# neel-dey/anatomix

Measured on AMD Instinct MI355X. Metric: 128^3 volumes/sec feature-extraction (6M UNet), higher is better.
Workload: dtype f16; 1 GPU; anatomix 6M UNet (ngf=16,num_downs=4) forward on sw_batch=4 windows of 1x128^3 (the predictor call of sliding_window_inference, BASELINE configs[1] / the metric); fp32 NCDHW in/out, 16-bit (f16) channels-last activations, fp32 accumulate; holds the 1e-3 tolerance against the fp32 reference in rel-L2 ONLY (max-norm 0.86e-3 .. 1.4e-3 by weight seed; the mode that holds both norms is value_strict); batch_per_gpu=4, window=128, parallelism=replicas x1 (no data-path collective)

## Files before the change

### anatomix_amd/csrc/amx_conv3d_zmarch.hip

```cpp
#include <stdio.h>
#include <stdlib.h>
#include <string.h>

#include "amx_device.h"

namespace amx {

typedef __attribute__((address_space(1))) const void* gptr_t;
typedef __attribute__((address_space(3))) void* lptr_t;

template <int NCK, int QT, int TY, int TX, int R>
struct ZmCfg {
  static constexpr int NC = 8, TZ = 2;
  static constexpr int NL = 2 * NCK;
  static constexpr int HY = TY + 2, HX = TX + 2, HVP = HY * HX;
  static constexpr int PPL = ((HVP * 16 + 255) / 256) * 256;
  static constexpr int PLSZ = NL * PPL;
  static constexpr int FLAGOFF = R * PLSZ;
  static constexpr int LDS_BYTES = R * PLSZ + 64;
  static constexpr int XT = TX / 16;
  static constexpr int WPQ = NC / QT;
  static constexpr int NDMA = (HVP + 63) / 64;
  static_assert(WPQ == (TY / 2) * XT, "each consumer wave owns a 2 x 2 x 16 voxel block per step");
  static_assert(R - 4 > TZ, "ring must hold more than one step of prefetch");
  static constexpr bool VMCNT_OK = R * NDMA <= 60;
  static_assert(NL <= 8 && LDS_BYTES <= 160 * 1024, "ring must fit the LDS");
};

template <int QT, int TY, int TX, int OUTMODE>
struct ZmStage {
  static constexpr int CB = 32 * QT;
  static constexpr int CS = 2 * TY * TX * 4 + 64;
  static constexpr int BYTES = OUTMODE == 0 ? 2 * TY * TX * CB : 16 * QT * CS;
  static constexpr int NB = OUTMODE == 0 ? 2 : 1;
  static constexpr int TOTAL = NB * BYTES;
};

struct StemIn {
  const char* src;
  long long sn, sz, sy;
  long long offs[16];
  int use_offs;
  const char* wpk;
  const float* bias;
  int act;
  float slope;
};

template <int TY, int TX>
struct ZmStemCfg {
  static constexpr int HY = TY + 2, HX = TX + 2, HVP = HY * HX;
  static constexpr int IY = HY + 2, IX = HX + 2, IVP = IY * IX;
  static constexpr int RS = (TX + 8) * 2;
  static constexpr int CPSZ = IY * RS;
  static constexpr int IPLSZ = ((2 * CPSZ + 8 + 63) / 64) * 64;
  static constexpr int DUMMY = IPLSZ - 8;
  static constexpr int RC = 16;
  static constexpr int SW = 40;
  static constexpr int STGSZ = ((IY * SW * 4 + 255) / 256) * 256;
  static constexpr int RSTG = 8;
  static constexpr int NLD = (IVP + 63) / 64;
  static constexpr int BYTES = RC * IPLSZ + RSTG * STGSZ;
  static constexpr int NSW = 7;
  static constexpr int LEAD = 3;
  static constexpr int NT = 2 * HY + (2 * HY + 15) / 16;
  static constexpr bool OK = TX == 32 && IY == 12 && RSTG * 2 <= 60 && NLD == 7;
};

template <typename T, int NCK, int QT, int TY, int TX, int R, int OUTMODE, int NS, bool POOL, bool SPLIT = false, bool STEM = false>
__global__ __launch_bounds__((8 + (STEM ? ZmStemCfg<8, 32>::NSW + 1 : 2 * (SPLIT ? 2 : NCK)) + NS) * 64) void conv3d_k3_zmarch_kernel(const ConvParams p, int zseg, int nseg, const StemIn si) {
  static_assert(!SPLIT || (NCK == 1 && QT == 1 && NS == 0), "strict z-march: 16 -> 16, direct stores");
  static_assert(!STEM || (NCK == 1 && !SPLIT && NS == 0 && OUTMODE == 0), "stem-fed z-march: 16 input channels, direct 16-bit stores");
  constexpr int NCKP = SPLIT ? 2 : NCK;
  typedef ZmCfg<NCKP, QT, TY, TX, R> C;
  typedef ZmStage<QT, TY, TX, OUTMODE> SG;
  typedef typename Ops<T>::vec8 vec8;
  constexpr int HX = C::HX, PPL = C::PPL, PLSZ = C::PLSZ, XT = C::XT, NDMA = C::NDMA, NL = C::NL, NC = C::NC, TZ = C::TZ;
  constexpr int STAGEOFF = C::FLAGOFF + 128;
  static_assert(NS == 0 || NS == 2, "one storer wave per output plane of a step");
  static_assert(NS == 0 || STAGEOFF + SG::TOTAL <= 160 * 1024, "ring + staging tile must fit the LDS");

  extern __shared__ __attribute__((aligned(16))) char smem[];

  const int tid = threadIdx.x, lane = tid & 63;
  const int wave = __builtin_amdgcn_readfirstlane(tid >> 6);

  int b = blockIdx.x;
  const int nb = gridDim.x;
  if ((nb & 7) == 0) b = (b & 7) * (nb >> 3) + (b >> 3);
  const int bx = b % p.nbx;
  b /= p.nbx;
  const int by = b % p.nby;
  b /= p.nby;
  const int sg = b % nseg;
  const int n = b / nseg;
  const int y0 = by * TY, x0 = bx * TX;
  const int zs = sg * zseg;
  const int ze = (zs + zseg < p.D) ? zs + zseg : p.D;
  const int nplanes = ze - zs + 2;
  const int nsteps = (ze - zs + TZ - 1) / TZ;

  int* ready = (int*)(smem + C::FLAGOFF);
  int* done = (int*)(smem + C::FLAGOFF + 32);
  int* staged = (int*)(smem + C::FLAGOFF + 64);
  int* stored = (int*)(smem + C::FLAGOFF + 96);
  if (tid < ((NS || STEM) ? 32 : 16))
    ((int*)(smem + C::FLAGOFF))[tid] = (STEM && (tid < 8 || tid >= 24)) ? ((tid & 7) == 7 ? 0x7fffffff : (tid & 7)) : 0;
  if constexpr (STEM) {
    typedef ZmStemCfg<TY, TX> SC;
    static_assert(SC::OK && STAGEOFF + SC::BYTES <= 160 * 1024, "stem-fed geometry; ring + input rings must fit the LDS");
    for (int i = tid; i < SC::RC * SC::IPLSZ / 4; i += (NC + SC::NSW + 1) * 64) ((int*)(smem + STAGEOFF))[i] = 0;
  }
  __syncthreads();

  if (NS && wave >= NC + NL) {
    const int w = wave - NC - NL;
    const unsigned a_staged = lds_addr(staged), a_stored = lds_addr(stored + w);
    if constexpr (OUTMODE == 0) {
      constexpr int NR = TY * QT;
      const char* sbase = smem + STAGEOFF + w * TY * TX * SG::CB + lane * 16;
      char* gbase = p.out + (long long)n * p.on + (long long)y0 * p.oy + (long long)x0 * p.ox + lane * 16;
      for (int s = 0; s < nsteps; ++s) {
        while (__builtin_amdgcn_readfirstlane(flag_min8_asm(a_staged)) < s + 1) __builtin_amdgcn_s_sleep(1);
        uint4 v[NR];
#pragma unroll
        for (int r = 0; r < NR; ++r) v[r] = *(const uint4*)(sbase + (s % SG::NB) * SG::BYTES + r * 1024);
        asm volatile("s_waitcnt lgkmcnt(0)" ::: "memory");
        flag_store_asm(a_stored, s + 1);
        const int zo = zs + s * TZ + w;
        if (zo >= ze || (p.dbg & 4)) continue;
        char* dst = gbase + (long long)zo * p.oz;
#pragma unroll
        for (int r = 0; r < NR; ++r) *(uint4*)(dst + (long long)(r / QT) * p.oy + (r % QT) * 1024) = v[r];
      }
    } else {
      constexpr int NCH = 16 * QT;
      const int y = lane >> 3, xq = lane & 7;
      const char* sbase = smem + STAGEOFF + (w * TY + y) * (TX * 4) + xq * 16;
      float* gbase = p.out32 + (long long)n * p.pn + (long long)(y0 + y) * p.py + x0 + xq * 4;
      for (int s = 0; s < nsteps; ++s) {
        while (__builtin_amdgcn_readfirstlane(flag_min8_asm(a_staged)) < s + 1) __builtin_amdgcn_s_sleep(1);
        float4 v[NCH];
#pragma unroll
        for (int c = 0; c < NCH; ++c) v[c] = *(const float4*)(sbase + c * SG::CS);
        asm volatile("s_waitcnt lgkmcnt(0)" ::: "memory");
        flag_store_asm(a_stored, s + 1);
        const int zo = zs + s * TZ + w;
        if (zo >= ze || (p.dbg & 4)) continue;
        float* dst = gbase + (long long)zo * p.pz;
        if (p.wmap) {
          const float4 wg = *(const float4*)(p.wmap + ((long long)zo * p.H + y0 + y) * p.W + x0 + xq * 4);
#pragma unroll
          for (int c = 0; c < NCH; ++c) {
            const float4 old = *(const float4*)(dst + (long long)c * p.pc);
            v[c] = make_float4(old.x + wg.x * v[c].x, old.y + wg.y * v[c].y, old.z + wg.z * v[c].z, old.w + wg.w * v[c].w);
          }
        }
#pragma unroll
        for (int c = 0; c < NCH; ++c) *(float4*)(dst + (long long)c * p.pc) = v[c];
      }
    }
    return;
  }

  if constexpr (STEM) {
    if (wave >= NC) {
      typedef ZmStemCfg<TY, TX> SC;
      constexpr int RS = SC::RS, CPSZ = SC::CPSZ, IPLSZ = SC::IPLSZ, RC = SC::RC, RSTG = SC::RSTG, NLD = SC::NLD, IX = SC::IX, SW = SC::SW;
      constexpr int INOFF = STAGEOFF, STGOFF = STAGEOFF + RC * IPLSZ;
      int* landed = staged;
      int* inconv = stored;
      const int zlo = zs >= 2 ? zs - 2 : 0;
      const int zhi = ze + 1 <= p.D - 1 ? ze + 1 : p.D - 1;
      const int nin = zhi - zlo + 1;
      const char* src_n = si.src + (si.use_offs ? si.offs[n & 15] : (long long)n * si.sn);
      if (wave == NC + SC::NSW) {
        const int pr = lane / 10, pc = lane - pr * 10;
        const bool pvalid = lane < 60;
        int goff[2];
#pragma unroll
        for (int j = 0; j < 2; ++j) {
          int yy = y0 - 2 + pr + 6 * j, xx = x0 - 4 + 4 * pc;
          yy = yy < 0 ? 0 : (yy > p.H - 1 ? p.H - 1 : yy);
          xx = xx < 0 ? 0 : (xx > p.W - 4 ? p.W - 4 : xx);
          goff[j] = pvalid ? yy * (int)si.sy + xx * 4 : 0;
        }
        auto issue_plane = [&](int k) {
          const char* plane = src_n + (long long)(zlo + k) * si.sz;
          char* dstp = smem + STGOFF + (k % RSTG) * SC::STGSZ;
          if (pvalid) {
            __builtin_amdgcn_global_load_lds((gptr_t)(plane + goff[0]), (lptr_t)dstp, 16, 0, 0);
            __builtin_amdgcn_global_load_lds((gptr_t)(plane + goff[1]), (lptr_t)(dstp + 960), 16, 0, 0);
          }
        };
        int next_issue = 0, next_pub = 0, seen_conv = 0;
        const unsigned a_landed = lds_addr(landed);
#ifdef AMX_EXPERIMENT
        unsigned long long* ltr = (p.dbg & 8) && lane == 0 && blockIdx.x == 0 ? (unsigned long long*)p.stats + 1001 * 128 : nullptr;
        int lcount = 0;
#define AMX_LSTAMP() do { if (ltr && lcount < 128) ltr[lcount] = __builtin_readcyclecounter(); ++lcount; } while (0)
        AMX_LSTAMP();
#else
#define AMX_LSTAMP() do {} while (0)
#endif
        while (next_pub < nin) {
          while (next_issue < nin) {
            const int need = next_issue - RSTG + 1;
            if (seen_conv < need) seen_conv = __builtin_amdgcn_readfirstlane(flag_min8_asm(lds_addr(inconv)));
            if (seen_conv < need) break;
            issue_plane(next_issue++);
          }
          if (next_issue == next_pub) {
            __builtin_amdgcn_s_sleep(2);
            continue;
          }
          AMX_LSTAMP();
          WaitVm<2, RSTG - 1>::run(next_issue - next_pub - 1);
          AMX_LSTAMP();
          flag_store_asm(a_landed, ++next_pub);
          AMX_LSTAMP();
        }
        return;
      }
      constexpr int NSW = SC::NSW;
      const int w = wave - NC;
      const int li = lane & 15, g = lane >> 4;
      const vec8 w0 = *(const vec8*)(si.wpk + 4096 + lane * 16);
      typedef __attribute__((ext_vector_type(2))) unsigned u32x2;
      typedef __attribute__((ext_vector_type(4))) unsigned u32x4;
      u32x2 w1 = *(const u32x2*)(si.wpk + 4096 + 1024 + lane * 16);
      if (g) w1 = u32x2{0u, 0u};
      const f32x4 sbias = si.bias ? *(const f32x4*)(si.bias + g * 4) : f32x4{0.f, 0.f, 0.f, 0.f};
      asm volatile("s_waitcnt vmcnt(0)" ::: "memory");
      const float lo_clip = si.act == ACT_RELU ? 0.f : -__builtin_inff();
      const int r0 = 2 * g, r1 = 2 * g + 1;
      const int kz0 = r0 / 3, kz1 = r1 / 3;
      auto xpart = [&](int hx) -> int {
        const int v0 = reflect_clamp(x0 + hx - 1, p.W) - (x0 - 2) - 1;
        return (v0 & 1) * CPSZ + (v0 & ~1) * 2;
      };
      auto ytop = [&](int hy) -> int { return reflect_clamp(y0 + hy - 1, p.H) - (y0 - 2) - 1; };
      const int xA = xpart(li), xB = xpart(16 + li);
      const int d0 = __builtin_amdgcn_readfirstlane((ytop(0) - 0) * RS), d9 = __builtin_amdgcn_readfirstlane((ytop(9) - 9) * RS);
      const int wlane = (g >> 1) * PPL + (g & 1) * 8 + li * 16;
      int croff[2], cwoff[2];
#pragma unroll
      for (int c = 0; c < 2; ++c) {
        const int crow = 8 * c + (li >> 1);
        const bool cvalid = crow < C::HY;
        const int crc = cvalid ? crow : 0;
        croff[c] = ytop(crc) * RS + xpart(32 + (li & 1));
        cwoff[c] = cvalid ? (g >> 1) * PPL + (g & 1) * 8 + (crow * HX + 32 + (li & 1)) * 16 : (g >> 1) * PPL + C::HVP * 16 + (g & 1) * 8;
      }
      constexpr int NB = 4;
      float vmax = 0.f;
      int seen_in = 0, seen_done = 0;
      int myk = w, seen_landed = 0, seen_ready = 0;
      bool ibad = false;
      auto convert_plane = [&](int k) {
        while (seen_landed < k + 1) {
          seen_landed = flag_load(landed);
          if (seen_landed < k + 1) __builtin_amdgcn_s_sleep(1);
        }
        const int need_done = zlo + k - RC + 3 - zs;
        while (seen_ready < need_done) {
          seen_ready = __builtin_amdgcn_readfirstlane(flag_min8_asm(lds_addr(ready)));
          if (seen_ready < need_done) __builtin_amdgcn_s_sleep(1);
        }
        asm volatile("" ::: "memory");
        const int so = (k % RSTG) * SC::STGSZ, dof = ((zlo + k) % RC) * IPLSZ;
        int lane_o = lane;
        asm volatile("" : "+v"(lane_o));
#pragma unroll
        for (int j = 0; j < NLD; ++j) {
          const int hv = j * 64 + lane_o;
          const bool valid = hv < SC::IVP;
          const int hvc = valid ? hv : SC::IVP - 1;
          const int iy = hvc / IX, ix = hvc - iy * IX;
          const int ry = reflect_clamp(y0 + iy - 2, p.H) - (y0 - 2), rx = reflect_clamp(x0 + ix - 2, p.W) - (x0 - 4);
          const float f = *(const float*)(smem + STGOFF + so + (ry * SW + rx) * 4);
          if (RangeCheck<T>::on) ibad |= RangeCheck<T>::bad(f);
          const unsigned short hb = to_bits<T>(f);
          const int la = valid ? iy * RS + ix * 2 : SC::DUMMY;
          const int lb = (valid && ix > 0) ? CPSZ + iy * RS + (ix - 1) * 2 : SC::DUMMY;
          *(unsigned short*)(smem + INOFF + dof + la) = hb;
          *(unsigned short*)(smem + INOFF + dof + lb) = hb;
        }
        asm volatile("" ::: "memory");
        flag_store(inconv + w, k + NSW);
      };
#ifdef AMX_EXPERIMENT
      unsigned long long* str = (p.dbg & 8) && lane == 0 && blockIdx.x == 0 && w == 0 ? (unsigned long long*)p.stats + 1000 * 128 : nullptr;
      int scount = 0;
#define AMX_SSTAMP() do { if (str && scount < 128) str[scount] = __builtin_readcyclecounter(); ++scount; } while (0)
      AMX_SSTAMP();
#else
#define AMX_SSTAMP() do {} while (0)
#endif
      for (int q = w; q < nplanes; q += NSW) {
        const int z1 = reflect_clamp(zs - 1 + q, p.D);
        int zi[3];
#pragma unroll
        for (int kz = 0; kz < 3; ++kz) zi[kz] = reflect_clamp(z1 - 1 + kz, p.D);
        int zmax = zi[0] > zi[1] ? zi[0] : zi[1];
        zmax = zmax > zi[2] ? zmax : zi[2];
        {
          int kmax = zs + q - zlo + SC::LEAD;
          kmax = kmax < nin - 1 ? kmax : nin - 1;
          for (; myk <= kmax; myk += NSW) convert_plane(myk);
        }
        while (seen_in < zmax - zlo + 1) {
          seen_in = __builtin_amdgcn_readfirstlane(flag_min8_asm(lds_addr(inconv)));
          if (seen_in < zmax - zlo + 1) __builtin_amdgcn_s_sleep(1);
        }
        while (q >= R + TZ * seen_done) {
          seen_done = __builtin_amdgcn_readfirstlane(flag_min8_asm(lds_addr(done)));
          if (q >= R + TZ * seen_done) __builtin_amdgcn_s_sleep(1);
        }
        asm volatile("" ::: "memory");
        AMX_SSTAMP();
#ifdef AMX_EXPERIMENT
        if (p.dbg & 64) { flag_store(ready + w, q + NSW); AMX_SSTAMP(); AMX_SSTAMP(); continue; }
#endif
        int ib[3];
#pragma unroll
        for (int kz = 0; kz < 3; ++kz) ib[kz] = INOFF + (zi[kz] % RC) * IPLSZ;
        const int b0 = (kz0 == 0 ? ib[0] : (kz0 == 1 ? ib[1] : ib[2])) + (r0 % 3) * RS;
        const int b1 = (kz1 == 0 ? ib[0] : (kz1 == 1 ? ib[1] : ib[2])) + (r1 % 3) * RS;
        const int b8 = ib[2] + 2 * RS;
        int a0 = b0 + xA, a1 = b1 + xA, a8 = b8 + xA, c0 = b0 + xB, c1 = b1 + xB, c8 = b8 + xB;
        int wr = (q % R) * PLSZ + wlane;
        asm volatile("" : "+v"(a0), "+v"(a1), "+v"(a8), "+v"(c0), "+v"(c1), "+v"(c8), "+v"(wr));
        auto rd = [&](int addr) -> u32x2 {
          const unsigned* qq = (const unsigned*)(smem + addr);
          return u32x2{qq[0], qq[1]};
        };
        auto raddr = [&](int TI, int& r_0, int& r_1, int& r_8) {
          if (TI < 2 * C::HY) {
            const int row = TI >> 1, xt = TI & 1;
            const int d = (row == 0 ? d0 : (row == C::HY - 1 ? d9 : 0)) + row * RS;
            r_0 = (xt ? c0 : a0) + d; r_1 = (xt ? c1 : a1) + d; r_8 = (xt ? c8 : a8) + d;
          } else {
            const int c = TI - 2 * C::HY;
            r_0 = b0 + croff[c]; r_1 = b1 + croff[c]; r_8 = b8 + croff[c];
          }
        };
        auto waddr = [&](int TI) -> int {
          if (TI < 2 * C::HY) return wr + ((TI >> 1) * HX + 16 * (TI & 1)) * 16;
          return (q % R) * PLSZ + cwoff[TI - 2 * C::HY];
        };
        constexpr int NBT = (SC::NT + NB - 1) / NB;
        u32x4 fa[2][NB];
        u32x2 fe[2][NB];
        f32x4 sacc[2][NB];
        auto stage_a = [&](int bt) {
#pragma unroll
          for (int t = 0; t < NB; ++t) {
            if (bt * NB + t >= SC::NT) continue;
            int r_0, r_1, r_8;
            raddr(bt * NB + t, r_0, r_1, r_8);
            const u32x2 a = rd(r_0), bq = rd(r_1);
            fa[bt & 1][t] = u32x4{a[0], a[1], bq[0], bq[1]};
            fe[bt & 1][t] = rd(r_8);
          }
        };
        auto stage_b = [&](int bt) {
#pragma unroll
          for (int t = 0; t < NB; ++t)
            if (bt * NB + t < SC::NT) sacc[bt & 1][t] = Ops<T>::mfma(w0, __builtin_bit_cast(vec8, fa[bt & 1][t]), sbias);
#pragma unroll
          for (int t = 0; t < NB; ++t)
            if (bt * NB + t < SC::NT) sacc[bt & 1][t] = Ops<T>::mfma16(w1, fe[bt & 1][t], sacc[bt & 1][t]);
        };
        auto stage_c = [&](int bt) {
#pragma unroll
          for (int t = 0; t < NB; ++t) {
            if (bt * NB + t >= SC::NT) continue;
            float v[4];
#pragma unroll
            for (int j = 0; j < 4; ++j) v[j] = __builtin_amdgcn_fmed3f(sacc[bt & 1][t][j], lo_clip, __builtin_inff());
            if (RangeCheck<T>::on) {
              asm("v_max3_f32 %0, %1, |%2|, |%3|" : "=v"(vmax) : "v"(vmax), "v"(v[0]), "v"(v[1]));
              asm("v_max3_f32 %0, %1, |%2|, |%3|" : "=v"(vmax) : "v"(vmax), "v"(v[2]), "v"(v[3]));
            }
            *(uint2*)(smem + waddr(bt * NB + t)) = make_uint2(Ops<T>::pack2(v[0], v[1]), Ops<T>::pack2(v[2], v[3]));
          }
        };
        stage_a(0);
        if (NBT > 1) stage_a(1);
        __builtin_amdgcn_sched_barrier(0);
        stage_b(0);
        __builtin_amdgcn_sched_barrier(0);
#pragma unroll
        for (int bt = 0; bt < NBT; ++bt) {
          if (bt + 2 < NBT) stage_a(bt + 2);
          __builtin_amdgcn_sched_barrier(0);
          if (bt + 1 < NBT) stage_b(bt + 1);
          __builtin_amdgcn_sched_barrier(0);
          stage_c(bt);
          __builtin_amdgcn_sched_barrier(0);
        }
        AMX_SSTAMP();
        asm volatile("" ::: "memory");
        flag_store(ready + w, q + NSW);
        AMX_SSTAMP();
      }
      for (; myk < nin; myk += NSW) convert_plane(myk);
      if (RangeCheck<T>::on) raise_flag(p.oflow, ibad | !(vmax <= 65504.f));
      return;
    }
  }

  if (!STEM && wave >= NC) {
    static_assert(STEM || C::VMCNT_OK, "loader wave must not exceed the 6-bit vmcnt range");
    const int cp = wave - NC;
    int off[NDMA];
    bool valid[NDMA];
#pragma unroll
    for (int j = 0; j < NDMA; ++j) {
      const int hv = j * 64 + lane;
      const int hy = hv / HX, hx = hv - hy * HX;
      valid[j] = hv < C::HVP;
      off[j] = halo_coord(y0 + hy - 1, p.H, p.raw_halo) * (int)p.s0y + halo_coord(x0 + hx - 1, p.W, p.raw_halo) * (int)p.s0x + cp * 16;
    }
    const char* src_n = p.src0 + (long long)n * p.s0n;
    auto issue_plane = [&](int q) {
      const char* plane = src_n + (long long)halo_coord(zs - 1 + q, p.D, p.raw_halo) * p.s0z;
      char* dstp = smem + (q % R) * PLSZ + cp * PPL;
#pragma unroll
      for (int j = 0; j < NDMA; ++j)
        if (valid[j]) __builtin_amdgcn_global_load_lds((gptr_t)(plane + off[j]), (lptr_t)(dstp + j * 1024), 16, 0, 0);
    };
    int next_issue = 0, next_pub = 0;
    const unsigned a_ready = lds_addr(ready + cp), a_done = lds_addr(done);
    while (next_pub < nplanes) {
      if (next_issue < nplanes) {
        const int md = __builtin_amdgcn_readfirstlane(flag_min8_asm(a_done));
        int lim = R + TZ * md;
        lim = lim < nplanes ? lim : nplanes;
        while (next_issue < lim) issue_plane(next_issue++);
      }
      if (next_issue == next_pub) {
        __builtin_amdgcn_s_sleep(2);
        continue;
      }
      WaitVm<NDMA, R - 1>::run(next_issue - next_pub - 1);
      flag_store_asm(a_ready, ++next_pub);
    }
    return;
  }

  const int li = lane & 15, g = lane >> 4, hi = g >> 1;
  const int wq = wave / C::WPQ;
  const int wr = wave % C::WPQ;
  const int wrow = (wr / XT) * 2;
  const int wcx = wr % XT;
  vec8 wreg[NCKP][kSteps];
#pragma unroll
  for (int k = 0; k < NCKP; ++k)
#pragma unroll
    for (int s = 0; s < kSteps; ++s) wreg[k][s] = *(const vec8*)(p.wpk + ((k * kSteps + s) * QT + wq) * 1024 + lane * 16);
  const int cb = g * 4 * QT + wq * 4;
  f32x4 bias = f32x4{0.f, 0.f, 0.f, 0.f};
  if (p.bias) bias = *(const f32x4*)(p.bias + cb);
  asm volatile("s_waitcnt vmcnt(0)" ::: "memory");

  const int lanebase = (g & 1) * PPL + ((wrow * HX) + wcx * 16 + li) * 16;
  const int base_d1 = lanebase + hi * 16;
  const int base_dx = lanebase + hi * 16 * HX;
  const bool full_xy = (y0 + TY <= p.H) & (x0 + TX <= p.W);

  const int yl = y0 + wrow, xl = x0 + wcx * 16 + li;
  char* out_l = OUTMODE == 0 ? p.out + (long long)n * p.on + (long long)yl * p.oy + (long long)xl * p.ox + cb * 2 : nullptr;
  float* out32_l = OUTMODE == 1 ? p.out32 + (long long)n * p.pn + (long long)cb * p.pc + (long long)yl * p.py + xl : nullptr;
  constexpr bool WIDE = OUTMODE == 0 && NS == 0 && QT == 1;
  char* out_w = WIDE ? p.out + (long long)n * p.on + (long long)(yl + (g & 1)) * p.oy + (long long)xl * p.ox + (g >> 1) * 16 : nullptr;
  const bool vec_planar = OUTMODE == 1 && !(p.W & 3) && !(p.py & 3) && !(p.pz & 3) && !(p.pc & 3) && !(p.pn & 3) &&
                          !((size_t)p.out32 & 15) && !((size_t)p.wmap & 15);
  float* out32_q = OUTMODE == 1 ? p.out32 + (long long)n * p.pn + (long long)(cb + (li & 3)) * p.pc + (long long)yl * p.py +
                                      x0 + wcx * 16 + (li & ~3)
                                : nullptr;
  char* out2_l = (OUTMODE == 0 && POOL) ? p.out2 + (long long)n * p.qn + (long long)(yl >> 1) * p.qy +
                                               (long long)(xl >> 1) * p.qx + cb * 2
                                          : nullptr;

  bool bad = false;
  unsigned long long* trace = (p.dbg & 8) && (wave == 0 || wave == 4) && lane == 0 && blockIdx.x < 500
                                  ? (unsigned long long*)p.stats + ((long long)blockIdx.x * 2 + (wave >> 2)) * 128 : nullptr;
  int tcount = 0;
#define AMX_ZSTAMP()                                                             \
  do {                                                                           \
    if (trace && tcount < 128) trace[tcount] = __builtin_readcyclecounter();     \
    ++tcount;                                                                    \
  } while (0)
  AMX_ZSTAMP();
  for (int s = 0; s < nsteps; ++s) {
    {
      int need = TZ * s + TZ + 2;
      need = need < nplanes ? need : nplanes;
      static_assert(NL <= 4 && C::FLAGOFF % 16 == 0, "the ready flags are polled with one 16-byte read");
      if constexpr (STEM) {
        while (__builtin_amdgcn_readfirstlane(flag_min8_asm(lds_addr(ready))) < need) __builtin_amdgcn_s_sleep(1);
      } else {
        while (flag_min4<NL>(ready) < need) __builtin_amdgcn_s_sleep(1);
      }
      asm volatile("" ::: "memory");
    }

    AMX_ZSTAMP();
#ifdef AMX_EXPERIMENT
    if (s == 0 && wave >= 4 && wave < 8)
      for (int k = (p.dbg >> 16) & 255; k > 0; --k) __builtin_amdgcn_s_sleep(8);
#endif
    int b1[4], bx3[4];
#pragma unroll
    for (int pl = 0; pl < 4; ++pl) {
      const int sl = ((s * TZ + pl) % R) * PLSZ;
      b1[pl] = base_d1 + sl;
      bx3[pl] = base_dx + sl;
    }
    f32x4 acc[2][2];
#pragma unroll
    for (int tz = 0; tz < 2; ++tz)
#pragma unroll
      for (int cy = 0; cy < 2; ++cy) acc[tz][cy] = bias;

    for (int rep = (p.dbg >> 10) & 7; rep >= 0; --rep)
    if (!(p.dbg & 2)) {
      if constexpr ((NCKP > 1 && !SPLIT) || STEM) {
        constexpr int PER = 4 * 6 + 8, NU = NCKP * PER, NSLOT = 4;
        int slo[4];
#pragma unroll
        for (int pl = 0; pl < 4; ++pl) slo[pl] = __builtin_amdgcn_readfirstlane(((s * TZ + pl) % R) * PLSZ);
        const int tail_lo = lanebase + (2 * HX + 2) * 16;
        auto src = [&](int i) -> const vec8* {
          const int ps = i / PER, j = i % PER, koff = ps * 2 * PPL;
          if (j < 24) {
            const int pl = j / 6, f = j % 6;
            return f < 4 ? (const vec8*)(smem + base_d1 + (slo[pl] + koff + (f * HX) * 16))
                         : (const vec8*)(smem + base_dx + (slo[pl] + koff + ((f - 4) * HX + 2) * 16));
          }
          const int t = j - 24, tz = t >> 2, cy = (t >> 1) & 1, which = t & 1;
          if (which) return (const vec8*)(smem + tail_lo + (slo[tz + 2] + koff + (cy * HX) * 16));
          return (const vec8*)(smem + tail_lo + ((hi ? slo[tz + 1] : slo[tz]) + koff + (cy * HX) * 16));
        };
        auto use = [&](int i, const vec8& frag) {
          const int ps = i / PER, j = i % PER;
          const int k = SPLIT ? 0 : ps;
          const bool both = SPLIT && ps == 0;
          auto mm = [&](const int widx, f32x4 a) {
            a = Ops<T>::mfma(wreg[k][widx], frag, a);
            if (both) a = Ops<T>::mfma(wreg[NCKP - 1][widx], frag, a);
            return a;
          };
          if (j < 24) {
            const int pl = j / 6, f = j % 6;
#pragma unroll
            for (int tz = 0; tz < 2; ++tz) {
              const int kz = pl - tz;
              if (kz < 0 || kz > 2) continue;
              if (f < 4) {
#pragma unroll
                for (int cy = 0; cy < 2; ++cy) {
                  const int ky = f - cy;
                  if (ky >= 0 && ky < 3) acc[tz][cy] = mm(kz * 3 + ky, acc[tz][cy]);
                }
              } else {
                acc[tz][f - 4] = mm(9 + kz, acc[tz][f - 4]);
              }
            }
          } else {
            const int t = j - 24, tz = t >> 2, cy = (t >> 1) & 1, which = t & 1;
            acc[tz][cy] = mm(12 + which, acc[tz][cy]);
          }
        };
        vec8 S[NSLOT];
#pragma unroll
        for (int i = 0; i < NSLOT; ++i) S[i] = *src(i);
#pragma clang loop unroll(full)
        for (int i = 0; i < NU; ++i) {
          use(i, S[i % NSLOT]);
          if (i + NSLOT < NU) S[i % NSLOT] = *src(i + NSLOT);
          __builtin_amdgcn_sched_barrier(0);
        }
      } else {
#pragma unroll
        for (int ps = 0; ps < NCKP; ++ps) {
          const int k = SPLIT ? 0 : ps;
          const bool both = SPLIT && ps == 0;
          const int koff = ps * 2 * PPL;
          auto mm = [&](const int widx, const vec8& frag, f32x4 a) {
            a = Ops<T>::mfma(wreg[k][widx], frag, a);
            if (both) a = Ops<T>::mfma(wreg[NCKP - 1][widx], frag, a);
            return a;
          };
          constexpr bool DB = NCKP == 1;
          vec8 F[DB ? 2 : 1][4], H[DB ? 2 : 1][2];
          auto load_plane = [&](int buf, int pl) {
  #pragma unroll
            for (int r = 0; r < 4; ++r) F[buf][r] = *(const vec8*)(smem + b1[pl] + koff + (r * HX) * 16);
  #pragma unroll
            for (int cy = 0; cy < 2; ++cy) H[buf][cy] = *(const vec8*)(smem + bx3[pl] + koff + (cy * HX + 2) * 16);
          };
          auto mma_plane = [&](int buf, int pl) {
  #pragma unroll
            for (int tz = 0; tz < 2; ++tz) {
              const int kz = pl - tz;
              if (kz < 0 || kz > 2) continue;
  #pragma unroll
              for (int ky = 0; ky < 3; ++ky)
  #pragma unroll
                for (int cy = 0; cy < 2; ++cy) acc[tz][cy] = mm(kz * 3 + ky, F[buf][cy + ky], acc[tz][cy]);
  #pragma unroll
              for (int cy = 0; cy < 2; ++cy) acc[tz][cy] = mm(9 + kz, H[buf][cy], acc[tz][cy]);
            }
          };
          if (DB) {
            load_plane(0, 0);
  #pragma unroll
            for (int pl = 0; pl < 4; ++pl) {
              if (pl + 1 < 4) load_plane((pl + 1) & 1, pl + 1);
              __builtin_amdgcn_sched_barrier(0);
              mma_plane(pl & 1, pl);
            }
          } else {
  #pragma unroll
            for (int pl = 0; pl < 4; ++pl) {
              load_plane(0, pl);
              mma_plane(0, pl);
            }
          }
  #pragma unroll
          for (int tz = 0; tz < 2; ++tz) {
            const int sl0 = ((s * TZ + tz) % R) * PLSZ, sl1 = ((s * TZ + tz + 1) % R) * PLSZ, sl2 = ((s * TZ + tz + 2) % R) * PLSZ;
            const int bz = lanebase + (hi ? sl1 : sl0) + koff + (2 * HX + 2) * 16;
            const int b0 = lanebase + sl2 + koff + (2 * HX + 2) * 16;
  #pragma unroll
            for (int cy = 0; cy < 2; ++cy) {
              const vec8 s0 = *(const vec8*)(smem + bz + (cy * HX) * 16);
              const vec8 s1 = *(const vec8*)(smem + b0 + (cy * HX) * 16);
              acc[tz][cy] = mm(12, s0, acc[tz][cy]);
              acc[tz][cy] = mm(13, s1, acc[tz][cy]);
            }
          }
        }
      }
      }
    asm volatile("s_waitcnt lgkmcnt(0)" ::: "memory");
    flag_store(done + wave, s + 1);
    AMX_ZSTAMP();

    if (p.dbg & 4) {
      if (NS) flag_store(staged + wave, s + 1);
      continue;
    }
    if constexpr (NS > 0) {
      if (s >= SG::NB)
        while (flag_min2(stored) < s + 1 - SG::NB) __builtin_amdgcn_s_sleep(1);
      asm volatile("" ::: "memory");
    }
    act_inplace<4>(&acc[0][0], p.act, p.slope);
    float pooled[4] = {-3.0e38f, -3.0e38f, -3.0e38f, -3.0e38f};
#pragma unroll
    for (int tz = 0; tz < 2; ++tz) {
      const int zo = zs + s * TZ + tz;
      if (WIDE && (SPLIT || !(p.dbg & 32))) {
        unsigned pk[2][2], pl[SPLIT ? 2 : 1][2];
#pragma unroll
        for (int cy = 0; cy < 2; ++cy) {
          float v[4];
#pragma unroll
          for (int j = 0; j < 4; ++j) {
            float f = acc[tz][cy][j];
              if (RangeCheck<T>::on) bad |= RangeCheck<T>::bad(f);
            v[j] = f;
            pooled[j] = f > pooled[j] ? f : pooled[j];
          }
          pk[cy][0] = (unsigned)to_bits<T>(v[0]) | ((unsigned)to_bits<T>(v[1]) << 16);
          pk[cy][1] = (unsigned)to_bits<T>(v[2]) | ((unsigned)to_bits<T>(v[3]) << 16);
          if constexpr (SPLIT) {
            float r[4];
#pragma unroll
            for (int j = 0; j < 4; ++j) r[j] = v[j] - (float)(T)v[j];
            pl[cy][0] = (unsigned)to_bits<T>(r[0]) | ((unsigned)to_bits<T>(r[1]) << 16);
            pl[cy][1] = (unsigned)to_bits<T>(r[2]) | ((unsigned)to_bits<T>(r[3]) << 16);
          }
        }
        const auto s0 = __builtin_amdgcn_permlane16_swap(pk[0][0], pk[1][0], false, false);
        const auto s1 = __builtin_amdgcn_permlane16_swap(pk[0][1], pk[1][1], false, false);
        unsigned l0a = 0, l0b = 0, l1a = 0, l1b = 0;
        if constexpr (SPLIT) {
          const auto t0 = __builtin_amdgcn_permlane16_swap(pl[0][0], pl[1][0], false, false);
          const auto t1 = __builtin_amdgcn_permlane16_swap(pl[0][1], pl[1][1], false, false);
          l0a = t0[0]; l0b = t0[1]; l1a = t1[0]; l1b = t1[1];
        }
        if (zo >= ze) continue;
        if (!full_xy && !((yl + (g & 1) < p.H) & (xl < p.W))) continue;
        *(uint4*)(out_w + (long long)zo * p.oz) = make_uint4(s0[0], s1[0], s0[1], s1[1]);
        if constexpr (SPLIT) *(uint4*)(out_w + (long long)zo * p.oz + p.Cout * 2) = make_uint4(l0a, l1a, l0b, l1b);
        continue;
      }
#pragma unroll
      for (int cy = 0; cy < 2; ++cy) {
        float v[4];
#pragma unroll
        for (int j = 0; j < 4; ++j) {
          float f = acc[tz][cy][j];
          if (OUTMODE == 0 && RangeCheck<T>::on) bad |= RangeCheck<T>::bad(f);
          v[j] = f;
          pooled[j] = f > pooled[j] ? f : pooled[j];
        }
        if constexpr (NS > 0) {
          if (OUTMODE == 0) {
            char* dst = smem + STAGEOFF + (s % SG::NB) * SG::BYTES + (((tz * TY + wrow + cy) * TX) + wcx * 16 + li) * SG::CB + cb * 2;
            *(uint2*)dst = make_uint2((unsigned)to_bits<T>(v[0]) | ((unsigned)to_bits<T>(v[1]) << 16),
                                      (unsigned)to_bits<T>(v[2]) | ((unsigned)to_bits<T>(v[3]) << 16));
          } else {
            quad_transpose4(v, li);
            char* dst = smem + STAGEOFF + (cb + (li & 3)) * SG::CS + ((tz * TY + wrow + cy) * TX + wcx * 16 + (li & ~3)) * 4;
            *(float4*)dst = make_float4(v[0], v[1], v[2], v[3]);
          }
          continue;
        }
        if (zo >= ze) continue;
        if (!full_xy && !((yl + cy < p.H) & (xl < p.W))) continue;
        if (OUTMODE == 0) {
          char* dst = out_l + (long long)zo * p.oz + cy * p.oy;
          *(uint2*)dst = make_uint2((unsigned)to_bits<T>(v[0]) | ((unsigned)to_bits<T>(v[1]) << 16),
                                    (unsigned)to_bits<T>(v[2]) | ((unsigned)to_bits<T>(v[3]) << 16));
        } else if (vec_planar) {
          quad_transpose4(v, li);
          float* dst = out32_q + (long long)zo * p.pz + cy * p.py;
          float4 o = make_float4(v[0], v[1], v[2], v[3]);
          if (p.wmap) {
            const float4 wg = *(const float4*)(p.wmap + ((long long)zo * p.H + yl + cy) * p.W + x0 + wcx * 16 + (li & ~3));
            const float4 old = *(const float4*)dst;
            o = make_float4(old.x + wg.x * o.x, old.y + wg.y * o.y, old.z + wg.z * o.z, old.w + wg.w * o.w);
          }
          *(float4*)dst = o;
        } else {
          float* dst = out32_l + (long long)zo * p.pz + cy * p.py;
          if (p.wmap) {
            const float wgt = p.wmap[((long long)zo * p.H + yl + cy) * p.W + xl];
#pragma unroll
            for (int j = 0; j < 4; ++j) dst[(long long)j * p.pc] += wgt * v[j];
          } else {
#pragma unroll
            for (int j = 0; j < 4; ++j) dst[(long long)j * p.pc] = v[j];
          }
        }
      }
    }
    if constexpr (NS > 0) {
      asm volatile("" ::: "memory");
      flag_store(staged + wave, s + 1);
    }
    if constexpr (OUTMODE == 0 && POOL) {
      float pm[4];
#pragma unroll
      for (int j = 0; j < 4; ++j) {
        const float o = dpp_quad<0xB1>(pooled[j]);
        pm[j] = pooled[j] > o ? pooled[j] : o;
      }
      const int zp = (zs + s * TZ) >> 1;
      if (!(li & 1) && zs + s * TZ + 1 < ze && (full_xy || ((yl + 1 < p.H) & (xl + 1 < p.W)))) {
        char* dst = out2_l + (long long)zp * p.qz;
        *(uint2*)dst = make_uint2((unsigned)to_bits<T>(pm[0]) | ((unsigned)to_bits<T>(pm[1]) << 16),
                                  (unsigned)to_bits<T>(pm[2]) | ((unsigned)to_bits<T>(pm[3]) << 16));
        if constexpr (SPLIT) {
          float r[4];
#pragma unroll
          for (int j = 0; j < 4; ++j) r[j] = pm[j] - (float)(T)pm[j];
          *(uint2*)(dst + p.Cout * 2) = make_uint2((unsigned)to_bits<T>(r[0]) | ((unsigned)to_bits<T>(r[1]) << 16),
                                                   (unsigned)to_bits<T>(r[2]) | ((unsigned)to_bits<T>(r[3]) << 16));
        }
      }
    }
    AMX_ZSTAMP();
  }
  if (OUTMODE == 0 && RangeCheck<T>::on) raise_flag(p.oflow, bad);
}

static thread_local char g_kernel_name3[64] = "";
const char* last_conv_zm_kernel_name() { return g_kernel_name3; }

template <typename T, int NCK, int QT, int TY, int R, int OUTMODE, int NS, bool POOL = false, bool SPLIT = false, int TX = 32, bool STEM = false>
static hipError_t launch_zm_ns(ConvParams p, hipStream_t st, const StemIn& si = StemIn{}) {
  if constexpr (OUTMODE == 0 && NS == 0 && !POOL && !STEM)
    if (p.out2) return launch_zm_ns<T, NCK, QT, TY, R, OUTMODE, NS, true, SPLIT, TX, STEM>(p, st, si);
  constexpr int TZ = 2;
  typedef ZmCfg<SPLIT ? 2 : NCK, QT, TY, TX, R> C;
  constexpr int LDS = STEM ? C::FLAGOFF + 128 + ZmStemCfg<TY, TX>::BYTES : NS ? C::FLAGOFF + 128 + ZmStage<QT, TY, TX, OUTMODE>::TOTAL : C::LDS_BYTES;
  if (STEM)
    snprintf(g_kernel_name3, sizeof g_kernel_name3, "conv3d_k3_zmarch<%s,stem1->16->16,%dx%dx%d,c8+st%d+ld1,r%d/%d%s>",
             __is_same(T, f16) ? "f16" : "bf16", TZ, TY, TX, ZmStemCfg<TY, TX>::NSW, R, ZmStemCfg<TY, TX>::RC, p.out2 ? ",pool" : "");
  else
  snprintf(g_kernel_name3, sizeof g_kernel_name3, "conv3d_k3_zmarch<%s%s,%d->%d,%dx%dx%d,c8+l%d+s%d,r%d,o%d%s>",
           __is_same(T, f16) ? "f16" : "bf16", SPLIT ? "x2" : "", 16 * NCK, 16 * QT, TZ, TY, TX, C::NL, NS, R, OUTMODE,
           p.out2 ? ",pool" : "");
  auto kern = conv3d_k3_zmarch_kernel<T, NCK, QT, TY, TX, R, OUTMODE, NS, POOL, SPLIT, STEM>;
  static amx::DeviceOnce attr_once;
  if (!attr_once.done()) {
    hipError_t e = hipFuncSetAttribute((const void*)kern, hipFuncAttributeMaxDynamicSharedMemorySize, LDS);
    if (e != hipSuccess) return e;
    attr_once.set();
  }
  static int dbg = -1;
  if (dbg < 0) {
    const char* e = exp_env("AMX_DBG");
    dbg = e ? atoi(e) : 0;
    if (exp_env("AMX_TRACE")) dbg |= 8;
  }
  p.dbg = dbg;
  p.nby = (p.H + TY - 1) / TY;
  p.nbx = (p.W + TX - 1) / TX;
  const int tiles = p.nby * p.nbx * p.N;
  int nseg, zseg;
  pick_z_segments(tiles, p.D, TZ, 256 * (LDS <= 80 * 1024 ? 2 : 1), &zseg, &nseg);
  static unsigned long long* trace_buf = nullptr;
  if (p.dbg & 8) {
    if (!trace_buf && hipMalloc((void**)&trace_buf, 1024 * 128 * 8) != hipSuccess) return hipErrorOutOfMemory;
    (void)hipMemsetAsync(trace_buf, 0, 1024 * 128 * 8, st);
    p.stats = (float*)trace_buf;
  }
  hipLaunchKernelGGL(kern, dim3((unsigned)(tiles * nseg)), dim3((8 + (STEM ? ZmStemCfg<TY, TX>::NSW + 1 : C::NL) + NS) * 64), LDS, st, p, zseg, nseg, si);
  if (p.dbg & 8) {
    static int printed = 0;
    (void)hipStreamSynchronize(st);
    if (printed++ == 3) {
      static unsigned long long hostbuf[1024 * 128];
      (void)hipMemcpy(hostbuf, trace_buf, sizeof hostbuf, hipMemcpyDeviceToHost);
      const int wgs[4] = {0, 77, 255, 500};
      for (int wi = 0; wi < (STEM ? 4 : 3); ++wi)
        for (int half = 0; half < 2; ++half) {
          const unsigned long long* tr = hostbuf + ((long long)wgs[wi] * 2 + half) * 128;
          fprintf(stderr, "[trace %s wg %d wave %d] wait/sweep/epilogue:", g_kernel_name3, wgs[wi], half * 4);
          for (int k = 1; k + 2 < 128 && tr[k + 2]; k += 3)
            fprintf(stderr, " %llu/%llu/%llu", tr[k] - tr[k - 1], tr[k + 1] - tr[k], tr[k + 2] - tr[k + 1]);
          fprintf(stderr, "\n");
        }
    }
  }
  return hipGetLastError();
}

template <int QT, int TY, int OUTMODE>
static bool zm_can_stage(const ConvParams& p) {
  static int off = -1;
  if (off < 0) off = exp_env("AMX_NO_STORERS") ? 1 : 0;
  if (off || p.H % TY || p.W % 32) return false;
  if (OUTMODE == 0)
    return p.ox == 32 * QT && !((size_t)p.out & 15) && !(p.oy & 15) && !(p.oz & 15) && !(p.on & 15);
  static int aligned_only = -1;
  if (aligned_only < 0) aligned_only = exp_env("AMX_STAGE_ALIGNED_ONLY") ? 1 : 0;
  if (aligned_only) return !(p.py & 3) && !(p.pz & 3) && !(p.pc & 3) && !(p.pn & 3) && !((size_t)p.out32 & 15) && !((size_t)p.wmap & 15);
  return !((size_t)p.out32 & 3) && !((size_t)p.wmap & 3);
}

template <typename T, int NCK, int QT, int TY, int R, int OUTMODE>
static hipError_t launch_zm(const ConvParams& p, hipStream_t st) {
  static int stage16 = -1;
  if (stage16 < 0) stage16 = exp_env("AMX_STAGE16") ? 1 : 0;
  if constexpr (NCK == 1)
    if ((OUTMODE == 1 || (stage16 && !p.out2)) && zm_can_stage<QT, TY, OUTMODE>(p)) return launch_zm_ns<T, NCK, QT, TY, R, OUTMODE, 2>(p, st);
  return launch_zm_ns<T, NCK, QT, TY, R, OUTMODE, 0>(p, st);
}

bool conv_zmarch_eligible(const ConvParams& p) {
  static int off = -1;
  if (off < 0) off = exp_env("AMX_NO_ZMARCH") ? 1 : 0;
  if (off || p.src0_f32c1 || p.C1 != 0 || p.W < 32 || p.H < 8 || p.D < 8) return false;
  if (p.C0 == 16 && p.Cout == 16) return true;
  if (p.out32) return false;
  return (p.C0 == 16 || p.C0 == 32) && p.Cout == 32;
}

bool conv_zmarch_can_pool(const ConvParams& p) {
  static int off = -1;
  if (off < 0) off = exp_env("AMX_NO_POOLFUSE") ? 1 : 0;
  return !off && conv_zmarch_eligible(p) && !p.out32 && !(p.D & 1) && !(p.H & 1) && !(p.W & 1);
}

bool conv_zmarch_eligible_split(const ConvParams& p) {
  static int off = -1;
  if (off < 0) off = exp_env("AMX_NO_ZMARCH_SPLIT") ? 1 : 0;
  return !off && conv_zmarch_eligible(p) && p.C0 == 16 && p.Cout == 16;
}
bool conv_zmarch_can_pool_split(const ConvParams& p) { return conv_zmarch_can_pool(p) && conv_zmarch_eligible_split(p); }

bool conv_zmarch_stem_eligible(const ConvParams& p, int precision) {
  static int off = -1;
  if (off < 0) off = exp_env("AMX_NO_STEMFUSE") ? 1 : 0;
  return !off && precision < 2 && p.C0 == 16 && p.C1 == 0 && p.Cout == 16 && !p.out32 && !p.raw_halo && p.W >= 32 && !(p.W % 32) && !(p.H % 8) &&
         !(p.D & 1) && p.D >= 8 && p.ox == 32 && (p.ocs == 0 || p.ocs == 32);
}
hipError_t launch_conv_zmarch_stem(const ConvParams& p, const float* x, long long xs_n, long long xs_z, long long xs_y, const long long* x_offs,
                                   const void* stem_wpk, const float* stem_bias, int stem_act, float stem_slope, int precision, hipStream_t st) {
  if (stem_act != ACT_NONE && stem_act != ACT_RELU) return hipErrorInvalidValue;
  if ((precision != 0 && precision != 1) || (x_offs && p.N > 16)) return hipErrorInvalidValue;
  StemIn si;
  memset(&si, 0, sizeof si);
  si.src = (const char*)x; si.sn = xs_n; si.sz = xs_z; si.sy = xs_y;
  if (x_offs) {
    si.use_offs = 1;
    for (int i = 0; i < p.N; ++i) si.offs[i] = x_offs[i] * 4;
  }
  si.wpk = (const char*)stem_wpk; si.bias = stem_bias; si.act = stem_act; si.slope = stem_slope;
  if (precision == 0) return launch_zm_ns<f16, 1, 1, 8, 10, 0, 0, false, false, 32, true>(p, st, si);
  return launch_zm_ns<bf16, 1, 1, 8, 10, 0, 0, false, false, 32, true>(p, st, si);
}

hipError_t launch_conv_zmarch(const ConvParams& p, int precision, hipStream_t st) {
  const bool planar = p.out32 != nullptr;
  if (precision >= 2) {
    if (p.C0 != 16 || p.Cout != 16) return hipErrorInvalidValue;
    if (precision == 2) return planar ? launch_zm_ns<f16, 1, 1, 8, 7, 1, 0, false, true>(p, st) : launch_zm_ns<f16, 1, 1, 8, 7, 0, 0, false, true>(p, st);
    return planar ? launch_zm_ns<bf16, 1, 1, 8, 7, 1, 0, false, true>(p, st) : launch_zm_ns<bf16, 1, 1, 8, 7, 0, 0, false, true>(p, st);
  }
  if (p.Cout == 16) {
    if (precision == 0) return planar ? launch_zm<f16, 1, 1, 8, 10, 1>(p, st) : launch_zm<f16, 1, 1, 8, 10, 0>(p, st);
    return planar ? launch_zm<bf16, 1, 1, 8, 10, 1>(p, st) : launch_zm<bf16, 1, 1, 8, 10, 0>(p, st);
  }
  if (p.C0 == 16) return precision == 0 ? launch_zm<f16, 1, 2, 4, 10, 0>(p, st) : launch_zm<bf16, 1, 2, 4, 10, 0>(p, st);
  return precision == 0 ? launch_zm<f16, 2, 2, 4, 10, 0>(p, st) : launch_zm<bf16, 2, 2, 4, 10, 0>(p, st);
}

}
```

Before: 2996 volumes/s.

## Trim zmarch register pressure: compile out debug flags, bias in LDS, split output addressing

Makes the debug flag a compile-time zero in non-experiment builds so the dbg branches fold away. For the 32-channel pooled variant, the bias moves into LDS and is reloaded each step instead of staying in registers. Per-lane 64-bit output pointers become a uniform base plus a 32-bit lane offset. The z-segment split now uses the runtime occupancy query instead of an LDS-size rule. The aim is to cut VGPR pressure and scalar overhead, at the cost of an extra LDS read per step and a different grid split when occupancy differs from the old rule.

```diff
diff --git a/anatomix_amd/csrc/amx_conv3d_zmarch.hip b/anatomix_amd/csrc/amx_conv3d_zmarch.hip
--- a/anatomix_amd/csrc/amx_conv3d_zmarch.hip
+++ b/anatomix_amd/csrc/amx_conv3d_zmarch.hip
@@ -84,6 +84,11 @@
 
   const int tid = threadIdx.x, lane = tid & 63;
   const int wave = __builtin_amdgcn_readfirstlane(tid >> 6);
+#ifdef AMX_EXPERIMENT
+  const int dbg = p.dbg;
+#else
+  constexpr int dbg = 0;
+#endif
 
   int b = blockIdx.x;
   const int nb = gridDim.x;
@@ -111,6 +116,10 @@
     static_assert(SC::OK && STAGEOFF + SC::BYTES <= 160 * 1024, "stem-fed geometry; ring + input rings must fit the LDS");
     for (int i = tid; i < SC::RC * SC::IPLSZ / 4; i += (NC + SC::NSW + 1) * 64) ((int*)(smem + STAGEOFF))[i] = 0;
   }
+  constexpr bool BIAS_LDS = NCK == 2 && POOL;
+  static_assert(!BIAS_LDS || (NS == 0 && !STEM && !SPLIT), "the bias takes the staging area");
+  if constexpr (BIAS_LDS)
+    if (tid < 16 * QT) ((float*)(smem + STAGEOFF))[tid] = p.bias ? p.bias[tid] : 0.f;
   __syncthreads();
 
   if (NS && wave >= NC + NL) {
@@ -128,7 +137,7 @@
         asm volatile("s_waitcnt lgkmcnt(0)" ::: "memory");
         flag_store_asm(a_stored, s + 1);
         const int zo = zs + s * TZ + w;
-        if (zo >= ze || (p.dbg & 4)) continue;
+        if (zo >= ze || (dbg & 4)) continue;
         char* dst = gbase + (long long)zo * p.oz;
 #pragma unroll
         for (int r = 0; r < NR; ++r) *(uint4*)(dst + (long long)(r / QT) * p.oy + (r % QT) * 1024) = v[r];
@@ -146,7 +155,7 @@
         asm volatile("s_waitcnt lgkmcnt(0)" ::: "memory");
         flag_store_asm(a_stored, s + 1);
         const int zo = zs + s * TZ + w;
-        if (zo >= ze || (p.dbg & 4)) continue;
+        if (zo >= ze || (dbg & 4)) continue;
         float* dst = gbase + (long long)zo * p.pz;
         if (p.wmap) {
           const float4 wg = *(const float4*)(p.wmap + ((long long)zo * p.H + y0 + y) * p.W + x0 + xq * 4);
@@ -196,7 +205,7 @@
         int next_issue = 0, next_pub = 0, seen_conv = 0;
         const unsigned a_landed = lds_addr(landed);
 #ifdef AMX_EXPERIMENT
-        unsigned long long* ltr = (p.dbg & 8) && lane == 0 && blockIdx.x == 0 ? (unsigned long long*)p.stats + 1001 * 128 : nullptr;
+        unsigned long long* ltr = (dbg & 8) && lane == 0 && blockIdx.x == 0 ? (unsigned long long*)p.stats + 1001 * 128 : nullptr;
         int lcount = 0;
 #define AMX_LSTAMP() do { if (ltr && lcount < 128) ltr[lcount] = __builtin_readcyclecounter(); ++lcount; } while (0)
         AMX_LSTAMP();
@@ -290,7 +299,7 @@
         flag_store(inconv + w, k + NSW);
       };
 #ifdef AMX_EXPERIMENT
-      unsigned long long* str = (p.dbg & 8) && lane == 0 && blockIdx.x == 0 && w == 0 ? (unsigned long long*)p.stats + 1000 * 128 : nullptr;
+      unsigned long long* str = (dbg & 8) && lane == 0 && blockIdx.x == 0 && w == 0 ? (unsigned long long*)p.stats + 1000 * 128 : nullptr;
       int scount = 0;
 #define AMX_SSTAMP() do { if (str && scount < 128) str[scount] = __builtin_readcyclecounter(); ++scount; } while (0)
       AMX_SSTAMP();
@@ -320,7 +329,7 @@
         asm volatile("" ::: "memory");
         AMX_SSTAMP();
 #ifdef AMX_EXPERIMENT
-        if (p.dbg & 64) { flag_store(ready + w, q + NSW); AMX_SSTAMP(); AMX_SSTAMP(); continue; }
+        if (dbg & 64) { flag_store(ready + w, q + NSW); AMX_SSTAMP(); AMX_SSTAMP(); continue; }
 #endif
         int ib[3];
 #pragma unroll
@@ -462,7 +471,7 @@
     for (int s = 0; s < kSteps; ++s) wreg[k][s] = *(const vec8*)(p.wpk + ((k * kSteps + s) * QT + wq) * 1024 + lane * 16);
   const int cb = g * 4 * QT + wq * 4;
   f32x4 bias = f32x4{0.f, 0.f, 0.f, 0.f};
-  if (p.bias) bias = *(const f32x4*)(p.bias + cb);
+  if (!BIAS_LDS && p.bias) bias = *(const f32x4*)(p.bias + cb);
   asm volatile("s_waitcnt vmcnt(0)" ::: "memory");
 
   const int lanebase = (g & 1) * PPL + ((wrow * HX) + wcx * 16 + li) * 16;
@@ -471,7 +480,9 @@
   const bool full_xy = (y0 + TY <= p.H) & (x0 + TX <= p.W);
 
   const int yl = y0 + wrow, xl = x0 + wcx * 16 + li;
-  char* out_l = OUTMODE == 0 ? p.out + (long long)n * p.on + (long long)yl * p.oy + (long long)xl * p.ox + cb * 2 : nullptr;
+  const int xu = x0 + wcx * 16;
+  const long long obase = (long long)n * p.on + (long long)yl * p.oy + (long long)xu * p.ox;
+  const unsigned olane = (unsigned)(li * (int)p.ox + cb * 2);
   float* out32_l = OUTMODE == 1 ? p.out32 + (long long)n * p.pn + (long long)cb * p.pc + (long long)yl * p.py + xl : nullptr;
   constexpr bool WIDE = OUTMODE == 0 && NS == 0 && QT == 1;
   char* out_w = WIDE ? p.out + (long long)n * p.on + (long long)(yl + (g & 1)) * p.oy + (long long)xl * p.ox + (g >> 1) * 16 : nullptr;
@@ -480,12 +491,11 @@
   float* out32_q = OUTMODE == 1 ? p.out32 + (long long)n * p.pn + (long long)(cb + (li & 3)) * p.pc + (long long)yl * p.py +
                                       x0 + wcx * 16 + (li & ~3)
                                 : nullptr;
-  char* out2_l = (OUTMODE == 0 && POOL) ? p.out2 + (long long)n * p.qn + (long long)(yl >> 1) * p.qy +
-                                               (long long)(xl >> 1) * p.qx + cb * 2
-                                          : nullptr;
+  const long long qbase = (long long)n * p.qn + (long long)(yl >> 1) * p.qy + (long long)(xu >> 1) * p.qx;
+  const unsigned qlane = (unsigned)((li >> 1) * (int)p.qx + cb * 2);
 
   bool bad = false;
-  unsigned long long* trace = (p.dbg & 8) && (wave == 0 || wave == 4) && lane == 0 && blockIdx.x < 500
+  unsigned long long* trace = (dbg & 8) && (wave == 0 || wave == 4) && lane == 0 && blockIdx.x < 500
                                   ? (unsigned long long*)p.stats + ((long long)blockIdx.x * 2 + (wave >> 2)) * 128 : nullptr;
   int tcount = 0;
 #define AMX_ZSTAMP()                                                             \
@@ -510,7 +520,7 @@
     AMX_ZSTAMP();
 #ifdef AMX_EXPERIMENT
     if (s == 0 && wave >= 4 && wave < 8)
-      for (int k = (p.dbg >> 16) & 255; k > 0; --k) __builtin_amdgcn_s_sleep(8);
+      for (int k = (dbg >> 16) & 255; k > 0; --k) __builtin_amdgcn_s_sleep(8);
 #endif
     int b1[4], bx3[4];
 #pragma unroll
@@ -520,13 +530,14 @@
       bx3[pl] = base_dx + sl;
     }
     f32x4 acc[2][2];
+    if constexpr (BIAS_LDS) bias = *(const f32x4*)(smem + STAGEOFF + cb * 4);
 #pragma unroll
     for (int tz = 0; tz < 2; ++tz)
 #pragma unroll
       for (int cy = 0; cy < 2; ++cy) acc[tz][cy] = bias;
 
-    for (int rep = (p.dbg >> 10) & 7; rep >= 0; --rep)
-    if (!(p.dbg & 2)) {
+    for (int rep = (dbg >> 10) & 7; rep >= 0; --rep)
+    if (!(dbg & 2)) {
       if constexpr ((NCKP > 1 && !SPLIT) || STEM) {
         constexpr int PER = 4 * 6 + 8, NU = NCKP * PER, NSLOT = 4;
         int slo[4];
@@ -650,7 +661,7 @@
     flag_store(done + wave, s + 1);
     AMX_ZSTAMP();
 
-    if (p.dbg & 4) {
+    if (dbg & 4) {
       if (NS) flag_store(staged + wave, s + 1);
       continue;
     }
@@ -664,7 +675,7 @@
 #pragma unroll
     for (int tz = 0; tz < 2; ++tz) {
       const int zo = zs + s * TZ + tz;
-      if (WIDE && (SPLIT || !(p.dbg & 32))) {
+      if (WIDE && (SPLIT || !(dbg & 32))) {
         unsigned pk[2][2], pl[SPLIT ? 2 : 1][2];
 #pragma unroll
         for (int cy = 0; cy < 2; ++cy) {
@@ -725,7 +736,7 @@
         if (zo >= ze) continue;
         if (!full_xy && !((yl + cy < p.H) & (xl < p.W))) continue;
         if (OUTMODE == 0) {
-          char* dst = out_l + (long long)zo * p.oz + cy * p.oy;
+          char* dst = p.out + (obase + (long long)zo * p.oz + cy * p.oy) + olane;
           *(uint2*)dst = make_uint2((unsigned)to_bits<T>(v[0]) | ((unsigned)to_bits<T>(v[1]) << 16),
                                     (unsigned)to_bits<T>(v[2]) | ((unsigned)to_bits<T>(v[3]) << 16));
         } else if (vec_planar) {
@@ -764,7 +775,9 @@
       }
       const int zp = (zs + s * TZ) >> 1;
       if (!(li & 1) && zs + s * TZ + 1 < ze && (full_xy || ((yl + 1 < p.H) & (xl + 1 < p.W)))) {
-        char* dst = out2_l + (long long)zp * p.qz;
+        unsigned ql = qlane;
+        asm volatile("" : "+v"(ql));
+        char* dst = p.out2 + (qbase + (long long)zp * p.qz) + ql;
         *(uint2*)dst = make_uint2((unsigned)to_bits<T>(pm[0]) | ((unsigned)to_bits<T>(pm[1]) << 16),
                                   (unsigned)to_bits<T>(pm[2]) | ((unsigned)to_bits<T>(pm[3]) << 16));
         if constexpr (SPLIT) {
@@ -790,7 +803,9 @@
     if (p.out2) return launch_zm_ns<T, NCK, QT, TY, R, OUTMODE, NS, true, SPLIT, TX, STEM>(p, st, si);
   constexpr int TZ = 2;
   typedef ZmCfg<SPLIT ? 2 : NCK, QT, TY, TX, R> C;
-  constexpr int LDS = STEM ? C::FLAGOFF + 128 + ZmStemCfg<TY, TX>::BYTES : NS ? C::FLAGOFF + 128 + ZmStage<QT, TY, TX, OUTMODE>::TOTAL : C::LDS_BYTES;
+  constexpr int LDS = STEM ? C::FLAGOFF + 128 + ZmStemCfg<TY, TX>::BYTES : NS ? C::FLAGOFF + 128 + ZmStage<QT, TY, TX, OUTMODE>::TOTAL
+                    : NCK == 2 && POOL ? C::FLAGOFF + 128 + 64 * QT
+                               : C::LDS_BYTES;
   if (STEM)
     snprintf(g_kernel_name3, sizeof g_kernel_name3, "conv3d_k3_zmarch<%s,stem1->16->16,%dx%dx%d,c8+st%d+ld1,r%d/%d%s>",
              __is_same(T, f16) ? "f16" : "bf16", TZ, TY, TX, ZmStemCfg<TY, TX>::NSW, R, ZmStemCfg<TY, TX>::RC, p.out2 ? ",pool" : "");
@@ -815,15 +830,22 @@
   p.nby = (p.H + TY - 1) / TY;
   p.nbx = (p.W + TX - 1) / TX;
   const int tiles = p.nby * p.nbx * p.N;
+  const int threads = (8 + (STEM ? ZmStemCfg<TY, TX>::NSW + 1 : C::NL) + NS) * 64;
+  static int per_cu = 0;
+  if (!per_cu) {
+    int nb = 0;
+    if (hipOccupancyMaxActiveBlocksPerMultiprocessor(&nb, (const void*)kern, threads, LDS) != hipSuccess || nb < 1) nb = 1;
+    per_cu = nb < (LDS <= 80 * 1024 ? 2 : 1) ? nb : (LDS <= 80 * 1024 ? 2 : 1);
+  }
   int nseg, zseg;
-  pick_z_segments(tiles, p.D, TZ, 256 * (LDS <= 80 * 1024 ? 2 : 1), &zseg, &nseg);
+  pick_z_segments(tiles, p.D, TZ, 256 * per_cu, &zseg, &nseg);
   static unsigned long long* trace_buf = nullptr;
   if (p.dbg & 8) {
     if (!trace_buf && hipMalloc((void**)&trace_buf, 1024 * 128 * 8) != hipSuccess) return hipErrorOutOfMemory;
     (void)hipMemsetAsync(trace_buf, 0, 1024 * 128 * 8, st);
     p.stats = (float*)trace_buf;
   }
-  hipLaunchKernelGGL(kern, dim3((unsigned)(tiles * nseg)), dim3((8 + (STEM ? ZmStemCfg<TY, TX>::NSW + 1 : C::NL) + NS) * 64), LDS, st, p, zseg, nseg, si);
+  hipLaunchKernelGGL(kern, dim3((unsigned)(tiles * nseg)), dim3(threads), LDS, st, p, zseg, nseg, si);
   if (p.dbg & 8) {
     static int printed = 0;
     (void)hipStreamSynchronize(st);
```

New measurement: 3029 volumes/s (median of 6 runs). 1.01x the previous value.
